# kamperh/segmentalist

Hardware: AMD Instinct MI355X
Metric: Gibbs sweeps/sec (10k utts, D=100, K=1000) at 1/2/4/8 MI355X (higher is better)
Workload: dtype fp16 one-product filter + fp16x2 second stage, float32 reference arithmetic for the results; 1 GPU; SegmentalKMeansWordseg batch-synchronous sweep (BASELINE.json configs[2]); utterances=10000, landmarks_per_utt=20, n_slices_max=6, embeddings=1050000, D=100, K=1000, parallelism=utterance shards x1, ONE all-gather of the packed block statistics per sweep, collective=none (single process), sweep_launch=plain launches, corpus=one device holds all rows, device_memory_allocated_bytes_rank0=1237140992, components_after=815

## Files before the change

### segmentalist_amd/csrc/segk_score_hint.hip

```cpp
#include "segk_kmeans_dev.h"

#define SEGK_K1_NW 4
#define SEGK_HINT_CHUNK 8

#ifndef SEGK_K1_ABL
#define SEGK_K1_ABL 0
#endif

struct K1Set {
    const float *tiles;
    int n_tiles;
    int tpr, n_ranges;
    float2 *part;
    int grid;
};

struct HintArgs {
    const unsigned char *ximg;
    const int32_t *ids;
    int64_t row0, n;
    K1Set full, delta;
    int K_max;
    int dbg;
    unsigned long long *stamp;
    float *fb_w;
    unsigned int *fb_t;
    int fb_cur;
    const int32_t *remap;
    int32_t *zero_cnt, *pre_hdr;
    int64_t k1_groups;
    const float *xrows32;
    int64_t ld32;
    const float *means32;
    const int32_t *cand_k;
    const float *nxx;
    float4 *hint_out;
    int32_t *ctl;
    const int32_t *meanchg;
    float *snap_img;
};

#define SEGK_MEANCHG_BIT 0x40000000

#define SEGK_RS_DRAIN_QUAD(O_, AO, q_, FIRST)                                                                               \
    do {                                                                                                                     \
        float x1_, u_;                                                                                                       \
        if (FIRST) {                                                                                                         \
            const float t1_ = __builtin_amdgcn_fmed3f(m1[O_], AO[4 * (q_)], AO[4 * (q_) + 1]);                              \
            asm volatile("v_max3_f32 %2, %0, %4, %5\n\t"                                                                     \
                         "v_med3_f32 %3, %2, %6, %7\n\t"                                                                     \
                         "v_max3_f32 %0, %2, %6, %7\n\t"                                                                     \
                         "v_max3_f32 %1, %1, %8, %3"                                                                          \
                         : "+v"(m1[O_]), "+v"(m2[O_]), "=&v"(x1_), "=&v"(u_)                                                 \
                         : "v"(AO[4 * (q_)]), "v"(AO[4 * (q_) + 1]), "v"(AO[4 * (q_) + 2]), "v"(AO[4 * (q_) + 3]), "v"(t1_)); \
        } else {                                                                                                             \
            float t1_;                                                                                                       \
            asm volatile("v_med3_f32 %4, %0, %5, %6\n\t"                                                                     \
                         "v_max3_f32 %2, %0, %5, %6\n\t"                                                                     \
                         "v_med3_f32 %3, %2, %7, %8\n\t"                                                                     \
                         "v_max3_f32 %0, %2, %7, %8\n\t"                                                                     \
                         "v_max3_f32 %1, %1, %4, %3"                                                                          \
                         : "+v"(m1[O_]), "+v"(m2[O_]), "=&v"(x1_), "=&v"(u_), "=&v"(t1_)                                     \
                         : "v"(AO[4 * (q_)]), "v"(AO[4 * (q_) + 1]), "v"(AO[4 * (q_) + 2]), "v"(AO[4 * (q_) + 3]));         \
        }                                                                                                                    \
    } while (0)

template <int KS, int V>
__device__ __forceinline__ void hint_wave_rows(const HintArgs &H, const int32_t *map , int64_t w, int64_t n_w, bool skip_ok)
{
    constexpr int D = 16 * KS - 4 * V;
    constexpr int nfull = D & ~7, nblk = nfull >> 3, rem = D & 7;
    constexpr int NX = nblk + (rem ? 1 : 0);
    typedef float f32x4_t __attribute__((ext_vector_type(4)));
    typedef float f32x2_t __attribute__((ext_vector_type(2)));
    typedef const __attribute__((address_space(1))) f32x4_t *gptr_t;
    const int lane = threadIdx.x & 63, row = lane >> 1, h = lane & 1;
    auto pk_sub = [](f32x2_t a, f32x2_t b2) -> f32x2_t {
        f32x2_t d;
        asm("v_pk_add_f32 %0, %1, %2 neg_lo:[0,1] neg_hi:[0,1]" : "=v"(d) : "v"(a), "v"(b2));
        return d;
    };
    const int64_t n_steps = (H.n + 31) >> 5;
    if (H.dbg & 8) return;
    auto rid_of = [&](int64_t s_) -> int32_t {
        const int64_t p_ = s_ * 32 + row;
        return p_ < H.n ? (H.ids ? H.ids[p_] : (int32_t)(H.row0 + p_)) : -1;
    };
    auto step_body = [&](int64_t s, int32_t rid_c, int32_t hint, bool skip, auto &&mid) {
        f32x4_t xv[NX], mv[NX];
#pragma unroll
        for (int b = 0; b < NX; b++) { xv[b] = f32x4_t{0.f, 0.f, 0.f, 0.f}; mv[b] = xv[b]; }
        if (!skip) {
            int64_t r_any = rid_c >= 0 ? (int64_t)rid_c : (H.ids ? 0 : H.row0);
            if (H.dbg & 16) r_any &= 1023;
            const uintptr_t xa = (uintptr_t)(H.xrows32 + r_any * H.ld32);
            const uintptr_t ma = (uintptr_t)(H.means32 + (int64_t)(hint >= 0 ? hint : 0) * D);
#pragma unroll
            for (int b = 0; b < nblk; b++) xv[b] = *reinterpret_cast<gptr_t>(xa + 16u * h + 32u * b);
            if constexpr (rem != 0) xv[nblk] = *reinterpret_cast<gptr_t>(xa + 4u * nfull);
#pragma unroll
            for (int b = 0; b < nblk; b++) mv[b] = *reinterpret_cast<gptr_t>(ma + 16u * h + 32u * b);
            if constexpr (rem != 0) mv[nblk] = *reinterpret_cast<gptr_t>(ma + 4u * nfull);
        }
        const float nx = rid_c >= 0 ? H.nxx[rid_c] : 0.f;
        if (H.dbg & 64) __builtin_amdgcn_s_sleep(64);
        mid();
        f32x2_t rl = {0.f, 0.f}, rh = {0.f, 0.f};
#pragma unroll
        for (int b = 0; b < ((H.dbg & 32) ? 1 : nblk); b++) {
            const f32x2_t dl = pk_sub(mv[b].xy, xv[b].xy), dh = pk_sub(mv[b].zw, xv[b].zw);
            const f32x2_t tl = dl * dl, th = dh * dh;
            rl = b == 0 ? tl : rl + tl;
            rh = b == 0 ? th : rh + th;
        }
        float res = (rl.x + rl.y) + (rh.x + rh.y);
        const float ro = __shfl_xor(res, 1);
        res = (h == 0) ? res + ro : ro + res;
        if constexpr (rem != 0) {
            const f32x2_t dl = pk_sub(mv[nblk].xy, xv[nblk].xy), dh = pk_sub(mv[nblk].zw, xv[nblk].zw);
            const f32x2_t tl = dl * dl, th = dh * dh;
            res += tl.x;
            if (rem > 1) res += tl.y;
            if (rem > 2) res += th.x;
            if (rem > 3) res += th.y;
        }
        const float sc = -res;
        const int64_t p = s * 32 + row;
        if (h == 0 && p < H.n && !skip) H.hint_out[p] = make_float4(sc, 0.5f * (sc - nx), __int_as_float(rid_c >= 0 ? hint : -1), 0.f);
    };
    int n_skipped = 0;
    if (skip_ok) {
        constexpr int CH = SEGK_HINT_CHUNK, PPL = CH / 2;
        const int crow = lane & 31, chalf = lane >> 5;
        auto chunk_load = [&](int64_t s0, int32_t (&rd)[PPL], int32_t (&kp)[PPL], int32_t (&pzv)[PPL]) {
#pragma unroll
            for (int u = 0; u < PPL; u++) {
                const int64_t s_ = s0 + (int64_t)(2 * u + chalf) * n_w, p_ = s_ * 32 + crow;
                const bool in = s_ < n_steps && p_ < H.n;
                rd[u] = in ? (H.ids ? H.ids[p_] : (int32_t)(H.row0 + p_)) : -1;
                pzv[u] = in ? __float_as_int(H.hint_out[p_].z) : -2;
            }
#pragma unroll
            for (int u = 0; u < PPL; u++) kp[u] = rd[u] >= 0 ? H.cand_k[rd[u]] : -1;
        };
        for (int64_t s0 = w; s0 < n_steps; s0 += (int64_t)CH * n_w) {
            int32_t rd[PPL], hv[PPL];
            unsigned long long live[PPL];
            {
                int32_t kp[PPL], pzv[PPL];
                chunk_load(s0, rd, kp, pzv);
#pragma unroll
                for (int u = 0; u < PPL; u++) {
                    const int64_t s_ = s0 + (int64_t)(2 * u + chalf) * n_w;
                    const bool in = s_ < n_steps && s_ * 32 + crow < H.n;
                    int32_t hint = (rd[u] >= 0 && kp[u] >= 0 && kp[u] < H.K_max) ? map[kp[u]] : -1;
                    const bool mchg = hint >= 0 && (hint & SEGK_MEANCHG_BIT) != 0;
                    if (hint >= 0) hint &= ~SEGK_MEANCHG_BIT;
                    const bool skip = rd[u] >= 0 && hint >= 0 && !mchg && pzv[u] == hint;
                    hv[u] = skip ? (hint | SEGK_MEANCHG_BIT) : hint;
                    live[u] = __ballot(in && !skip);
                    n_skipped += __popcll(__ballot(skip));
                }
            }
#pragma unroll 1
            for (int i = 0; i < CH; i++) {
                const int64_t s_ = s0 + (int64_t)i * n_w;
                if (s_ >= n_steps) break;
                int32_t rd_s = rd[0], hv_s = hv[0];
                unsigned long long lv = live[0];
#pragma unroll
                for (int u = 1; u < PPL; u++)
                    if ((i >> 1) == u) { rd_s = rd[u]; hv_s = hv[u]; lv = live[u]; }
                const int sh = 32 * (i & 1);
                if ((unsigned)(lv >> sh) == 0u) continue;
                const int src = sh + row;
                const int32_t rid_c = __shfl(rd_s, src);
                int32_t hint = __shfl(hv_s, src);
                const bool skip = hint >= 0 && (hint & SEGK_MEANCHG_BIT) != 0;
                if (hint >= 0) hint &= ~SEGK_MEANCHG_BIT;
                step_body(s_, rid_c, rid_c >= 0 ? hint : -1, skip, [] {});
            }
        }
        if (n_skipped > 0 && lane == 0) atomicAdd(H.ctl + 3, n_skipped);
        return;
    }
    int64_t s = w;
    int32_t rid = -1, rid_n = -1, kprev = -1;
    if (s < n_steps) {
        rid = rid_of(s);
        if (s + n_w < n_steps) rid_n = rid_of(s + n_w);
        kprev = rid >= 0 ? H.cand_k[rid] : -1;
    }
    for (; s < n_steps; s += n_w) {
        int32_t hint = (rid >= 0 && kprev >= 0 && kprev < H.K_max) ? map[kprev] : -1;
        if (hint >= 0) hint &= ~SEGK_MEANCHG_BIT;
        step_body(s, rid, hint, false, [&] {
            rid = rid_n;
            kprev = rid >= 0 ? H.cand_k[rid] : -1;
            const int64_t s2 = s + 2 * n_w;
            rid_n = s2 < n_steps ? rid_of(s2) : -1;
        });
    }
}

struct XcdShare { int64_t lo, hi; };
__device__ __forceinline__ XcdShare k1_xcd_share(const HintArgs &H, int64_t total_groups, bool delta, bool record)
{
    const int lane = threadIdx.x & 63, x = lane & 7;
    const int cur = H.fb_cur, prev = (cur + 2) % 3, next = (cur + 1) % 3;
    const float wp = H.fb_w[prev * 8 + x];
    const unsigned int tp = H.fb_t ? H.fb_t[prev * 8 + x] : 0u;
    const bool ok = __all(tp > 0u && wp > 0.f);
    const float rate = ok ? wp / (float)tp : 0.f;
    float rsum = rate;
    rsum += __shfl_xor(rsum, 1);
    rsum += __shfl_xor(rsum, 2);
    rsum += __shfl_xor(rsum, 4);
    float w = !(wp > 0.f) ? 0.125f : ok ? 0.5f * wp + 0.5f * (rate / rsum) : wp;
    w = fminf(fmaxf(w, 0.0625f), 0.25f);
    float wsum = w;
    wsum += __shfl_xor(wsum, 1);
    wsum += __shfl_xor(wsum, 2);
    wsum += __shfl_xor(wsum, 4);
    double cum = 0.0;
    for (int y = 0; y < 8; y++) {
        const float wy = __shfl(w, y);
        if (y < x) cum += (double)wy;
    }
    const int64_t split = (int64_t)(cum * ((double)total_groups / (double)wsum));
    const int xcd = blockIdx.x & 7;
    XcdShare s;
    s.lo = __shfl(split, xcd);
    s.hi = xcd == 7 ? total_groups : __shfl(split, (xcd + 1) & 7);
    if (record && lane < 8) {
        H.fb_w[cur * 8 + x] = delta ? (wp > 0.f ? wp : 0.125f) : w / wsum;
        if (H.fb_t) {
            H.fb_t[next * 8 + x] = 0u;
            if (delta) H.fb_t[cur * 8 + x] = tp;
        }
    }
    return s;
}

template <int KS, int V>
__global__ __launch_bounds__(128 * SEGK_K1_NW, 1) void k_kmeans_top2_rs(HintArgs H)
{
    typedef _Float16 T;
    typedef SegkPiece::V8 V8;
    constexpr int P = 2, KP = KS * 16, NBLK = 2;
    constexpr int STRIDE = (KS * P * 256 + 32 + 1023) / 1024 * 1024;
    constexpr int TL = KS * 256 + 32;
    extern __shared__ __attribute__((aligned(16))) float lds[];
    const int tid = threadIdx.x, lane = tid & 63, wave = tid >> 6;
    const int j = lane & 31, h = lane >> 5;
    const int mw = H.ctl ? __builtin_amdgcn_readfirstlane(H.ctl[0]) : 0;
    const bool delta = (mw & SEGK_DELTA_MODE) != 0, skip_ok = (mw & SEGK_DELTA_SKIP) != 0;
    const K1Set S = delta ? H.delta : H.full;
    const int n_tiles = delta ? __builtin_amdgcn_readfirstlane(H.ctl[2]) : S.n_tiles;
    const int tpr = S.tpr, R = S.n_ranges, grid = S.grid;
    const float *tiles = S.tiles;
    float2 *part = S.part;
    if ((int)blockIdx.x >= grid) return;
    const int map_off = tpr * TL;
    const bool is_hint = wave >= SEGK_K1_NW;
    if (!is_hint) __builtin_amdgcn_s_setprio(2);
#ifdef SEGK_STAMP
    const unsigned long long st_k0 = __builtin_amdgcn_s_memtime(), st_r0 = __builtin_amdgcn_s_memrealtime();
#endif
    int range, wgr, n_wgr;
    const bool xcd_aware = (grid & 7) == 0 && ((grid >> 3) % R) == 0;
    if (xcd_aware) {
        const int xcd = blockIdx.x & 7, idx = blockIdx.x >> 3;
        range = idx % R;
        wgr = (idx / R) * 8 + xcd;
        n_wgr = grid / R;
    } else {
        n_wgr = grid / R;
        range = blockIdx.x % R;
        wgr = blockIdx.x / R;
    }
    const int t_lo = range * tpr;
    int nt = n_tiles - t_lo;
    if (nt > tpr) nt = tpr;
    const bool mm_on = wgr < n_wgr && nt > 0;
    if (nt < 1) nt = 1;
    const T *plane0 = (const T *)(H.ximg + SEGK_SP_HEADER);
    const int64_t total_groups = (H.n + 32 * NBLK - 1) / (32 * NBLK);
    int64_t n_groups = H.k1_groups < total_groups ? H.k1_groups : total_groups, n_slots = (int64_t)n_wgr * SEGK_K1_NW, g_first = (int64_t)wgr * SEGK_K1_NW + wave;
    const unsigned long long fb_t0 = __builtin_amdgcn_s_memrealtime();
    if (blockIdx.x == 0 && tid == 0) {
        if (H.zero_cnt) *H.zero_cnt = 0;
#pragma unroll
        for (int i = 0; i < 16; i++) H.pre_hdr[i] = 0;
    }
    const XcdShare share = k1_xcd_share(H, total_groups, delta, blockIdx.x == 0 && wave == 0);
    const bool fb = xcd_aware && H.fb_t != nullptr && !delta;
    if (fb) {
        n_slots = (int64_t)(n_wgr >> 3) * SEGK_K1_NW;
        g_first = share.lo + (int64_t)(wgr >> 3) * SEGK_K1_NW + wave;
        n_groups = share.hi;
    }

#define SEGK_RS_LOAD(g_, XB)                                                                                    \
    do {                                                                                                         \
        _Pragma("unroll") for (int b = 0; b < NBLK; b++) {                                                       \
            const int64_t r = (g_) * (32 * NBLK) + 32 * b + j;                                                   \
            int64_t rowid = -1;                                                                                  \
            if (r < H.n) rowid = H.ids ? (int64_t)H.ids[r] : H.row0 + r;                                         \
            if (rowid < 0) rowid = 0;           \
            const T *xp = plane0 + rowid * KP + 8 * h;                                                           \
            _Pragma("unroll") for (int s = 0; s < KS; s++) XB[b][s] = *reinterpret_cast<const V8 *>(xp + 16 * s); \
        }                                                                                                        \
    } while (0)

#define SEGK_RS_UNIT(XB, N_, AN, O_, AO, REFILL)                                                                     \
    do {                                                                                                              \
        _Pragma("unroll") for (int s = 0; s < KS; s++) {                                                              \
            asm volatile("" : "+v"(a[s]));                                                                            \
            AN = __builtin_amdgcn_mfma_f32_32x32x16_f16(a[s], XB[N_][s], s == 0 ? cs : AN, 0, 0, 0);                  \
            asm volatile("" : "+v"(AN));                                                                              \
            if (REFILL && !(SEGK_K1_ABL & 2)) {    \
                load_a(tn, s);                                                                                        \
                if (s == 0) load_cs(tn);                                                                              \
            }                                                                                                         \
            __builtin_amdgcn_sched_barrier(0);                                                                        \
                      \
            constexpr int SL = KS > 1 ? KS - 1 : 1;                                                                   \
            const int q_lo = KS > 1 ? ((s - 1) * 4 + SL - 1) / SL : 0, q_hi = KS > 1 ? (s * 4 + SL - 1) / SL : 4;     \
            if ((KS == 1 || s >= 1) && !(SEGK_K1_ABL & 1)) {                                                          \
                if (0 >= q_lo && 0 < q_hi) SEGK_RS_DRAIN_QUAD(O_, AO, 0, true);                                       \
                if (1 >= q_lo && 1 < q_hi) SEGK_RS_DRAIN_QUAD(O_, AO, 1, false);                                      \
                if (2 >= q_lo && 2 < q_hi) SEGK_RS_DRAIN_QUAD(O_, AO, 2, false);                                      \
                if (3 >= q_lo && 3 < q_hi) SEGK_RS_DRAIN_QUAD(O_, AO, 3, false);                                      \
            }                                                                                                         \
            __builtin_amdgcn_sched_barrier(0);                                                                        \
        }                                                                                                             \
    } while (0)

#define SEGK_RS_TILE(XB, t_)                                        \
    do {                                                            \
        const int tn = (t_) + 1 < nt ? (t_) + 1 : 0;      \
        SEGK_RS_UNIT(XB, 0, acc0, 1, acc1, false);                  \
        SEGK_RS_UNIT(XB, 1, acc1, 0, acc0, true);                   \
    } while (0)

#define SEGK_RS_GROUP(g_, XB)                                                                                             \
    do {                                                                                                                   \
        float m1[NBLK], m2[NBLK];                                                                                          \
        _Pragma("unroll") for (int b = 0; b < NBLK; b++) { m1[b] = NEG_INF_F; m2[b] = NEG_INF_F; }                         \
        f32x16 acc0, acc1;                                                                                                 \
        _Pragma("unroll") for (int q = 0; q < 16; q++) acc1[q] = NEG_INF_F;         \
        int t = 0;                                                                                                         \
        for (; t + 1 < nt; t += 2) {                                                                                       \
            SEGK_RS_TILE(XB, t);                                                                                           \
            SEGK_RS_TILE(XB, t + 1);                                                                                       \
        }                                                                                                                  \
        if (t < nt) SEGK_RS_TILE(XB, t);                                                                                   \
        SEGK_RS_DRAIN_QUAD(NBLK - 1, acc1, 0, true);                                                                       \
        SEGK_RS_DRAIN_QUAD(NBLK - 1, acc1, 1, false);                                                                      \
        SEGK_RS_DRAIN_QUAD(NBLK - 1, acc1, 2, false);                                                                      \
        SEGK_RS_DRAIN_QUAD(NBLK - 1, acc1, 3, false);                                                                      \
           \
          \
          \
        _Pragma("unroll") for (int b = 0; b < NBLK; b++) {                                                                 \
            const float o1 = __shfl_xor(m1[b], 32), o2 = __shfl_xor(m2[b], 32);                                            \
            pend1[b] = fmaxf(m1[b], o1);                                                                                   \
            pend2[b] = fmaxf(fminf(m1[b], o1), fmaxf(m2[b], o2));                                                          \
        }                                                                                                                  \
        pend_g = (g_);                                                                                                     \
    } while (0)

#define SEGK_RS_STORE()                                                                                                    \
    do {                                                                                                                   \
        if (pend_g >= 0) {                                                                                                 \
            _Pragma("unroll") for (int b = 0; b < NBLK; b++) {                                                             \
                const int64_t r = pend_g * (32 * NBLK) + 32 * b + j;                                                       \
                if (h == 0 && r < H.n && !(H.dbg & 1)) part[(int64_t)range * H.n + r] = make_float2(pend1[b], pend2[b]); \
            }                                                                                                              \
        }                                                                                                                  \
    } while (0)

    V8 a[KS];
    f32x16 cs;
    auto load_a = [&](int t, int s) { a[s] = *reinterpret_cast<const V8 *>((const T *)(lds + t * TL) + (s * 64 + lane) * 8); };
    auto load_cs = [&](int t) {
        const float *cv = lds + t * TL + KS * 256 + 4 * h;
#pragma unroll
        for (int q = 0; q < 4; q++) {
            const float4 c4 = *reinterpret_cast<const float4 *>(cv + 8 * q);
            cs[4 * q + 0] = c4.x; cs[4 * q + 1] = c4.y; cs[4 * q + 2] = c4.z; cs[4 * q + 3] = c4.w;
        }
    };
    int64_t g = g_first;
    float pend1[NBLK], pend2[NBLK];
    int64_t pend_g = -1;
    V8 xa[NBLK][KS];
    typedef __attribute__((address_space(3))) void *lptr_t;
    if (!is_hint && mm_on && g < n_groups && !(H.dbg & 4)) SEGK_RS_LOAD(g, xa);
#ifdef SEGK_STAMP
    const unsigned long long st_k1 = __builtin_amdgcn_s_memtime();
#endif
    {
        constexpr int MAXT = (160 * 1024 / (TL * 4)) < SEGK_HINT_MAX_TPR ? (160 * 1024 / (TL * 4)) : SEGK_HINT_MAX_TPR;
        constexpr int MAXB = MAXT * KS;
        constexpr int NWF = 2 * SEGK_K1_NW;
        constexpr int PER_W = (MAXB + NWF - 1) / NWF;
        const int n_blk = nt * KS;
        const int rot = (int)(((unsigned)wgr * 2654435761u) >> 8) % n_blk;
        const unsigned lds0 = __builtin_amdgcn_readfirstlane((unsigned)(uintptr_t)(lptr_t)lds);
#pragma unroll
        for (int u = 0; u < PER_W; u++) {
            int c = wave + u * NWF;
            if (mm_on && c < n_blk) {
                c += rot;
                if (c >= n_blk) c -= n_blk;
                const int t = __builtin_amdgcn_readfirstlane(c / KS), ks = __builtin_amdgcn_readfirstlane(c) - t * KS;
                const float *src = tiles + (int64_t)(t_lo + t) * STRIDE + ks * (P * 256) + lane * 4;
                const unsigned dst = lds0 + (unsigned)(t * TL + ks * 256) * 4u;
                unsigned keep_;
                asm volatile("s_mov_b32 %0, m0\n\ts_mov_b32 m0, %2\n\ts_nop 0\n\t"
                             "global_load_lds_dwordx4 %1, off\n\ts_mov_b32 m0, %0"
                             : "=&s"(keep_)
                             : "v"(src), "s"(dst)
                             : "memory");
            }
        }
        float4 cv4 = make_float4(0.f, 0.f, 0.f, 0.f);
        const bool has_c = mm_on && tid < nt * 8;
        if (has_c) cv4 = *reinterpret_cast<const float4 *>(tiles + (int64_t)(t_lo + (tid >> 3)) * STRIDE + KS * P * 256 + (tid & 7) * 4);
        int32_t *map_l = reinterpret_cast<int32_t *>(lds + map_off);
        for (int k = tid; k < H.K_max; k += 128 * SEGK_K1_NW) {
            int v = H.remap ? H.remap[k] : k;
            if (v < 0 || v >= H.K_max) v = -1;
            else if (H.full.tiles[(int64_t)(v >> 5) * STRIDE + KS * P * 256 + (v & 31)] < -1.0e37f) v = -1;
            if (skip_ok && v >= 0 && H.meanchg[v]) v |= SEGK_MEANCHG_BIT;
            map_l[k] = v;
        }
        if (has_c) *reinterpret_cast<float4 *>(lds + (tid >> 3) * TL + KS * 256 + (tid & 7) * 4) = cv4;
        static_assert(128 * SEGK_K1_NW >= MAXT * 8, "one thread per float4 of the constants");
    }
    asm volatile("s_waitcnt vmcnt(0)" ::: "memory");
    __syncthreads();
    if (is_hint) {
        if (H.ctl && !delta && mm_on && wgr == 0) {
            float4 *dst = reinterpret_cast<float4 *>(H.snap_img + 4 + (int64_t)t_lo * TL);
            const float4 *src = reinterpret_cast<const float4 *>(lds);
            for (int i = tid - 64 * SEGK_K1_NW; i < nt * (TL / 4); i += 64 * SEGK_K1_NW) dst[i] = src[i];
        }
        hint_wave_rows<KS, V>(H, reinterpret_cast<const int32_t *>(lds + map_off), (int64_t)blockIdx.x * SEGK_K1_NW + (wave - SEGK_K1_NW),
                              (int64_t)grid * SEGK_K1_NW, skip_ok);
        return;
    }
#ifdef SEGK_STAMP
    const unsigned long long st_k2 = __builtin_amdgcn_s_memtime();
#endif
    if (!mm_on || g >= n_groups || (H.dbg & 128)) return;
    if (H.dbg & 4) SEGK_RS_LOAD(g, xa);
#pragma unroll
    for (int s = 0; s < KS; s++) load_a(0, s);
    load_cs(0);
    V8 xb[NBLK][KS];
#ifdef SEGK_STAMP
    unsigned long long st_wait = 0, st_loop = 0, st_groups = 0;
    const unsigned long long st_begin = __builtin_amdgcn_s_memtime();
#define SEGK_ST(var) const unsigned long long var = __builtin_amdgcn_s_memtime()
#else
#define SEGK_ST(var) do { } while (0)
#endif
    for (;;) {
        SEGK_ST(s0);
        __builtin_amdgcn_s_waitcnt(0x0F70);
        SEGK_ST(s1);
        const int64_t g1 = g + n_slots;
        if (g1 < n_groups) SEGK_RS_LOAD(g1, xb);
        SEGK_RS_STORE();
        SEGK_ST(s2);
        SEGK_RS_GROUP(g, xa);
        SEGK_ST(s3);
#ifdef SEGK_STAMP
        st_wait += s1 - s0; st_loop += s3 - s2; st_groups++;
#endif
        if (g1 >= n_groups) break;
        SEGK_ST(s4);
        __builtin_amdgcn_s_waitcnt(0x0F70);
        SEGK_ST(s5);
        g = g1 + n_slots;
        if (g < n_groups) SEGK_RS_LOAD(g, xa);
        SEGK_RS_STORE();
        SEGK_ST(s6);
        SEGK_RS_GROUP(g1, xb);
        SEGK_ST(s7);
#ifdef SEGK_STAMP
        st_wait += s5 - s4; st_loop += s7 - s6; st_groups++;
#endif
        if (g >= n_groups) break;
    }
#ifdef SEGK_STAMP
    if (H.stamp && lane == 0) {
        unsigned long long *o = H.stamp + ((int64_t)blockIdx.x * SEGK_K1_NW + wave) * 8;
        o[0] = st_wait; o[1] = st_loop; o[2] = __builtin_amdgcn_s_memtime() - st_begin; o[3] = st_groups;
        o[4] = st_begin - st_k0; o[5] = st_r0; o[6] = __builtin_amdgcn_s_memrealtime(); o[7] = ((st_k1 - st_k0) << 32) | (st_k2 - st_k1);
    }
#endif
#undef SEGK_ST
    SEGK_RS_STORE();
    if (fb && lane == 0) atomicMax(&H.fb_t[H.fb_cur * 8 + (blockIdx.x & 7)], (unsigned int)(__builtin_amdgcn_s_memrealtime() - fb_t0));
#undef SEGK_RS_STORE
#undef SEGK_RS_GROUP
#undef SEGK_RS_TILE
#undef SEGK_RS_UNIT
#undef SEGK_RS_LOAD
}
#undef SEGK_RS_DRAIN_QUAD

template <int KS>
__global__ __launch_bounds__(SEGK_PREP_THREADS) void k_delta_prep(DeltaPrepArgs P)
{
    if ((int)blockIdx.x >= P.n_tiles) {
        delta_prep_means_rows(P, (int)blockIdx.x - P.n_tiles, (int)gridDim.x - P.n_tiles);
        return;
    }
    __shared__ DeltaPrepLds S;
    const int e_cur = ((const int *)P.tiles_hdr)[0];
    if (delta_prep_tile(P, KS, (int)blockIdx.x, e_cur, S)) delta_prep_mode(P, KS, e_cur, S);
}

struct HintMergeArgs {
    const float2 *part;
    const float4 *hint_out;
    int n_ranges;
    const float *tiles_hdr;
    const unsigned char *ximg;
    const int32_t *ctl;
    const float2 *part_delta;
    int32_t *lab_base;
    const int32_t *colchg;
    const int32_t *meanchg;
    int32_t *lab_last;
    int32_t *stats_host;
};

#define SEGK_MERGE_ROWS 6144
#define SEGK_MERGE_THREADS 1024
__global__ __launch_bounds__(SEGK_MERGE_THREADS) void k_hint_merge(ScoreArgs A, HintMergeArgs H, int KP, int64_t per, float *pre_thr, int64_t first_skipped)
{
    __shared__ int32_t ulist[SEGK_MERGE_ROWS];
    __shared__ float uthr[SEGK_MERGE_ROWS];
    __shared__ int32_t ucnt, ubase;
    const int tid = threadIdx.x, lane = tid & 63;
    if (tid == 0) ucnt = 0;
    const int mw = H.ctl ? H.ctl[0] : 0;
    const bool delta = (mw & SEGK_DELTA_MODE) != 0;
    const int n_chg = H.ctl ? H.ctl[1] : 0, n_packed = H.ctl ? H.ctl[2] : 0;
    if (H.stats_host && blockIdx.x == 0 && tid == 0) {
        H.stats_host[1] = n_chg;
        H.stats_host[2] = n_packed;
        H.stats_host[3] = H.ctl ? H.ctl[3] : 0;
        __hip_atomic_store(H.stats_host, H.ctl ? 1 + (delta ? 1 : 0) : 0, __ATOMIC_RELEASE, __HIP_MEMORY_SCOPE_SYSTEM);
    }
    __syncthreads();
    bool carry = false;
    if (delta && (mw & SEGK_DELTA_SKIP) != 0 && H.lab_last) {
        const int c_off = (KP / 16) * 512;
        bool bad = false;
        for (int k = tid; k < A.K_max; k += SEGK_MERGE_THREADS)
            if (H.meanchg[k] && !H.colchg[k])
                bad |= !(H.tiles_hdr[1024 + (int64_t)(k >> 5) * A.tile_stride + c_off + (k & 31)] < -1.0e37f);
        carry = __syncthreads_or(bad ? 1 : 0) == 0;
    }
    const int64_t p_lo = (int64_t)blockIdx.x * per, p_hi = p_lo + per < A.n ? p_lo + per : A.n;
    const int e_ab = ((const int *)H.ximg)[1] + ((const int *)H.tiles_hdr)[0];
    const float unscale = ldexpf(1.f, -e_ab), scale = ldexpf(1.f, e_ab);
    const float M = (float)(sqrt(*A.mnorm2) * (1.0 + 1e-6)) + 1e-30f;
    const float Em = H.tiles_hdr[1];
    constexpr int U = 5;
    for (int64_t p0 = p_lo; p0 < p_hi; p0 += SEGK_MERGE_THREADS * U) {
        int32_t rid[U];
        float4 ho[U];
        float t1[U], t2[U], xnb[U], xer[U], d1[U];
        int32_t last[U];
        bool cw[U];
#pragma unroll
        for (int j = 0; j < U; j++) {
            const int64_t p = p0 + j * SEGK_MERGE_THREADS + tid;
            rid[j] = -1;
            if (p < p_hi) rid[j] = A.ids ? A.ids[p] : (int32_t)(A.row0 + p);
        }
#pragma unroll
        for (int j = 0; j < U; j++) {
            const int64_t p = p0 + j * SEGK_MERGE_THREADS + tid;
            ho[j] = make_float4(0.f, 0.f, __int_as_float(-1), 0.f);
            t1[j] = NEG_INF_F; t2[j] = NEG_INF_F; xnb[j] = 0.f; xer[j] = 0.f;
            if (rid[j] >= 0) {
                ho[j] = H.hint_out[p];
                for (int r = 0; r < H.n_ranges; r++) {
                    const float2 pv = H.part[(int64_t)r * A.n + p];
                    const float n1 = fmaxf(t1[j], pv.x);
                    t2[j] = fmaxf(fminf(t1[j], pv.x), fmaxf(t2[j], pv.y));
                    t1[j] = n1;
                }
                xnb[j] = A.xnorm[rid[j]];
                xer[j] = A.xerr[rid[j]];
            }
            d1[j] = NEG_INF_F;
            last[j] = -2;
            cw[j] = false;
            if (rid[j] >= 0 && carry) {
                const int32_t hint = __float_as_int(ho[j].z);
                last[j] = H.lab_last[p];
                cw[j] = hint >= 0 && last[j] == hint && H.meanchg[hint] == 0;
            }
            if (rid[j] >= 0 && delta) {
                const int32_t hint = __float_as_int(ho[j].z);
                if (hint >= 0 && H.colchg[hint] && H.lab_base[p] == hint) {
                    t1[j] = t2[j];
                }
                if (n_packed > 0) {
                    const float2 pv = H.part_delta[p];
                    d1[j] = pv.x;
                    const float n1 = fmaxf(t1[j], pv.x);
                    t2[j] = fmaxf(fminf(t1[j], pv.x), fmaxf(t2[j], pv.y));
                    t1[j] = n1;
                }
            }
        }
#pragma unroll
        for (int j = 0; j < U; j++) {
            bool und = false;
            float thr = 0.f;
            int32_t keep = -1;
            if (rid[j] >= 0 && p0 + j * SEGK_MERGE_THREADS + tid >= first_skipped) {
                const int q2 = atomicAdd(A.cand.count, 1);
                if (q2 < A.amb_cap) A.cand.queue[q2] = rid[j];
            } else if (rid[j] >= 0) {
                const int32_t hint = __float_as_int(ho[j].z);
                und = true;
                const float tau = filter_tau_h1(xnb[j], M, A.D, xer[j], Em);
                float lower = t1[j];
                thr = t1[j] - tau * scale * 1.000001f;
                thr -= 4e-7f * fabsf(t1[j]);
                bool ok = false;
                if (hint >= 0) {
                    const float top1 = t1[j] * unscale, top2 = t2[j] * unscale;
                    const float u = 5.9604645e-8f;
                    const float e1 = (1.02f * (float)(KP + 16) + 16.f) * u * (xnb[j] * M + 0.5f * M * M);
                    const float rnd = 1.00001f * fminf((xnb[j] + xer[j]) * Em + xer[j] * M, 1.01f * 9.765625e-4f * xnb[j] * M);
                    const float s2 = xnb[j] + M;
                    const float dl = ((float)(A.D / 8 + 13) + 4.f) * u * s2 * s2;
                    ok = (top1 - top2 > tau) && (ho[j].y >= top1 - tau + (e1 + rnd + dl) * 1.0001f);
                    const bool carried = !ok && cw[j] && ho[j].y > d1[j] * unscale + (e1 + rnd + dl) * 1.0001f;
                    if (ok || carried) {
                        A.cand.k[rid[j]] = hint;
                        A.cand.s[rid[j]] = (double)ho[j].x;
                        und = false;
                        keep = hint;
                    }
                    lower = (ho[j].y - (e1 + rnd + dl) * 1.0001f) * scale;
                    lower -= 4e-7f * fabsf(lower);
                }
                if (H.lab_base && !delta) H.lab_base[p0 + j * SEGK_MERGE_THREADS + tid] = ok ? hint : -1;
                if (und && delta && n_chg > 0) {
                    if (hint < 0) {
                        und = false;
                        const int q2 = atomicAdd(A.cand.count, 1);
                        if (q2 < A.amb_cap) A.cand.queue[q2] = rid[j];
                    } else {
                        lower = fmaxf(lower, d1[j]);
                        thr = lower - tau * scale * 1.000001f;
                        thr -= 4e-7f * fabsf(lower);
                    }
                }
            }
            if (H.lab_last && rid[j] >= 0 && last[j] != keep) H.lab_last[p0 + j * SEGK_MERGE_THREADS + tid] = keep;
            const unsigned long long mask = __ballot(und);
            if (mask != 0ull) {
                const int before = __builtin_amdgcn_mbcnt_hi((unsigned)(mask >> 32), __builtin_amdgcn_mbcnt_lo((unsigned)mask, 0));
                int base = 0;
                if (lane == 0) base = atomicAdd(&ucnt, __popcll(mask));
                base = __shfl(base, 0);
                if (und) {
                    ulist[base + before] = rid[j];
                    uthr[base + before] = thr;
                }
            }
        }
    }
    __syncthreads();
    const int cnt = ucnt;
    if (cnt == 0) return;
    if (tid == 0) ubase = atomicAdd(A.pre_count, cnt);
    __syncthreads();
    const int base = ubase;
    for (int i = tid; i < cnt; i += SEGK_MERGE_THREADS) {
        const int q = base + i;
        const int32_t rid = ulist[i];
        if (q < A.pre_cap) {
            A.pre_queue[q] = rid;
            if (pre_thr) pre_thr[q] = uthr[i];
        } else {
            const int q2 = atomicAdd(A.cand.count, 1);
            if (q2 < A.amb_cap) A.cand.queue[q2] = rid;
        }
    }
}

struct HintLaunch {
    HintPlan lds;
    bool band;
    int grid;
    int64_t k1_groups;
    float *fb_w;
    unsigned int *fb_t;
    int fb_cur;
    float4 *hint_out;
    bool part_fresh;
};

static int hint_workspaces(segk_ctx *ctx, ScoreArgs &A, HintLaunch &L, hipStream_t st)
{
    if (int rc = segk_ws_grow(ctx, &ctx->pre_queue, &ctx->pre_cap, A.n, sizeof(int32_t) * (size_t)(A.n + 16), st)) return rc;
    A.pre_queue = ctx->pre_queue + 16;
    A.pre_count = ctx->pre_queue;
    A.pre_cap = (int)A.n;
    if (L.band)
        if (int rc = segk_ws_grow(ctx, &ctx->pre_thr, &ctx->pre_thr_cap, A.n, sizeof(float) * (size_t)A.n, st)) return rc;
    const size_t part_bytes = ((size_t)L.lds.n_ranges * (size_t)A.n * sizeof(float2) + 255) & ~(size_t)255;
    const size_t need_part = part_bytes + (size_t)A.n * sizeof(float4);
    L.part_fresh = ctx->hint_part_bytes < need_part;
    if (int rc = segk_ws_grow(ctx, &ctx->hint_part, &ctx->hint_part_bytes, need_part, need_part, st)) return rc;
    L.hint_out = (float4 *)((unsigned char *)ctx->hint_part + part_bytes);
    if (!ctx->hint_fb) {
        float init[3 * 8 + 3 * 8];
        SEGK_CHECK_HIP(hipMalloc(&ctx->hint_fb, sizeof(init)));
        for (int i = 0; i < 24; i++) init[i] = 0.125f;
        memset(init + 24, 0, 24 * sizeof(unsigned int));
        SEGK_CHECK_HIP(hipMemcpyAsync(ctx->hint_fb, init, sizeof(init), hipMemcpyHostToDevice, st));
        SEGK_CHECK_HIP(hipStreamSynchronize(st));
        ctx->hint_fb_launch = 0;
    }
    return SEGK_OK;
}

static void hint_plan_rows(segk_ctx *ctx, const ScoreArgs &A, HintLaunch &L)
{
    const int n_ranges = L.lds.n_ranges;
    const int64_t total_groups = (A.n + 63) / 64;
    L.fb_w = (float *)ctx->hint_fb;
    const bool fb_big = total_groups >= 192 * 64;
    L.fb_t = (segk_env_int("SEGK_HINT_BALANCE", 1) == 0 || !fb_big) ? nullptr : (unsigned int *)(L.fb_w + 24);
    L.fb_cur = (int)(ctx->hint_fb_launch++ % 3u);
    L.grid = (ctx->n_cu / n_ranges) * n_ranges;
    const int64_t steps = (A.n + 64 * SEGK_K1_NW - 1) / (64 * SEGK_K1_NW);
    if ((int64_t)L.grid / n_ranges > steps) L.grid = (int)steps * n_ranges;
    L.k1_groups = total_groups;
    if (!L.fb_t && !L.band) {
        const int64_t slots = (int64_t)(L.grid / n_ranges) * SEGK_K1_NW;
        const int64_t whole = slots > 0 ? (total_groups / slots) * slots : 0;
        if (whole > 0 && total_groups - whole <= 32) L.k1_groups = whole;
    }
}

struct DeltaBuf {
    int32_t *ctl;
    int32_t *colchg, *meanchg;
    float *snap_img;
    float *packed;
    float *snap_means;
    float2 *part;
    int32_t *lab_base;
    int32_t *lab_last;
    size_t zero_bytes;
};
static size_t delta_layout(unsigned char *b, int n_tiles, int K_max, int D, int64_t n, int stride, DeltaBuf *B)
{
    const size_t TL = (size_t)(segk_b3_kp(D) / 16) * 256 + 32;
    size_t off = 0;
    auto take = [&](size_t bytes) {
        unsigned char *p = b ? b + off : nullptr;
        off += (bytes + 255) & ~(size_t)255;
        return p;
    };
    B->ctl = (int32_t *)take(256);
    B->colchg = (int32_t *)take((size_t)n_tiles * 32 * 4);
    B->meanchg = (int32_t *)take((size_t)K_max * 4);
    B->snap_img = (float *)take(((size_t)n_tiles * TL + 4) * 4);
    B->packed = (float *)take((size_t)n_tiles * stride * 4);
    B->zero_bytes = off;
    B->snap_means = (float *)take((size_t)K_max * D * 4);
    B->part = (float2 *)take((size_t)n * 8);
    B->lab_base = (int32_t *)take((size_t)n * 4);
    B->lab_last = (int32_t *)take((size_t)n * 4);
    return off;
}

static int delta_cap(const HintPlan &lds)
{
    int cap = segk_env_int("SEGK_DELTA_CAP", lds.tpr);
    if (cap > lds.max_tiles) cap = lds.max_tiles;
    return cap < 1 ? 1 : cap;
}
static int delta_budget(int n_tiles) { return segk_env_int("SEGK_DELTA_BUDGET", n_tiles); }

static DeltaPrepArgs delta_prep_args(segk_ctx *ctx, const DeltaBuf &B, const float *tiles, int n_tiles, int stride, int K_max, int D,
                                     const float *means32, const int32_t *remap, const int32_t *K_dev, bool valid, int cap, int budget,
                                     int redo_seq = -1)
{
    DeltaPrepArgs P{};
    P.tiles_hdr = tiles; P.n_tiles = n_tiles; P.stride = stride;
    P.K_max = K_max; P.D = D; P.means32 = means32; P.remap = remap; P.K_dev = K_dev;
    P.valid = valid ? 1 : 0; P.hint_valid = valid ? 1 : 0; P.cap = cap;
    P.budget = budget;
    P.redo = redo_seq >= 0 ? 1 : 0;
    P.seq = redo_seq >= 0 ? redo_seq : (int)(ctx->delta_seq++ & 1u);
    P.ctl = B.ctl; P.colchg = B.colchg; P.meanchg = B.meanchg;
    P.snap_img = B.snap_img; P.packed = B.packed; P.snap_means = B.snap_means;
    return P;
}

bool segk_delta_prep_fold(segk_ctx *ctx, const segk_corpus *c, const segk_kmeans *m, const int32_t *remap, hipStream_t st, DeltaPrepArgs *P)
{
    *P = DeltaPrepArgs{};
    if (!ctx || ctx->delta_pending != 0 || !ctx->delta_valid || ctx->capturing || !ctx->delta_buf) return false;
    if (segk_env_int("SEGK_DELTA_PREP_FOLD", 1) == 0 || segk_env_int("SEGK_SCORE_DELTA", 1) == 0) return false;
    const void *key[4] = {c->Xb3, c->X32, m->tiles_b3, m->means};
    const int64_t key_n[5] = {0, c->n_emb, c->n_emb, m->K_max, c->D};
    if (memcmp(key, ctx->delta_key, sizeof(key)) != 0 || memcmp(key_n, ctx->delta_key_n, sizeof(key_n)) != 0) return false;
    const int n_tiles = segk_n_tiles(m->K_max), stride_sp = segk_sp_tile_stride(c->D, 2);
    HintPlan lds;
    if (n_tiles > 32 * SEGK_PREP_COLS || !segk_hint_plan(m->K_max, segk_b3_kp(c->D) / 16, n_tiles, &lds)) return false;
    DeltaBuf B{};
    if (ctx->delta_bytes != delta_layout(nullptr, n_tiles, m->K_max, c->D, c->n_emb, stride_sp, &B)) return false;
    delta_layout((unsigned char *)ctx->delta_buf, n_tiles, m->K_max, c->D, c->n_emb, stride_sp, &B);
    const int cap = delta_cap(lds), budget = delta_budget(n_tiles);
    *P = delta_prep_args(ctx, B, m->tiles_b3, n_tiles, stride_sp, m->K_max, c->D, (const float *)m->means, remap, m->K, true, cap, budget);
    ctx->delta_pending = 1;
    ctx->delta_pending_remap = remap; ctx->delta_pending_K = m->K; ctx->delta_pending_stream = (const void *)st;
    ctx->delta_pending_cap = cap; ctx->delta_pending_budget = budget; ctx->delta_pending_seq = P->seq;
    return true;
}

template <int KS>
static int launch_delta_prep(segk_ctx *ctx, const ScoreArgs &A, const int32_t *remap, const int32_t *K_dev, int64_t n_emb,
                             const HintLaunch &L, hipStream_t st, DeltaBuf *B, int *cap)
{
    *B = DeltaBuf{};
    *cap = 0;
    const int pending = ctx->delta_pending;
    ctx->delta_pending = 0;
    const bool delta_on = segk_env_int("SEGK_SCORE_DELTA", 1) != 0 && L.band && A.ids == nullptr && A.n_tiles <= 32 * SEGK_PREP_COLS;
    const void *key[6] = {A.X32, A.xrows32, A.tiles, A.means32, A.cand.k, A.cand.s};
    const int64_t key_n[5] = {A.row0, A.n, n_emb, A.K_max, A.D};
    bool state_valid = delta_on && !L.part_fresh && ctx->delta_valid && memcmp(key, ctx->delta_key, sizeof(key)) == 0 &&
                       memcmp(key_n, ctx->delta_key_n, sizeof(key_n)) == 0;
    ctx->delta_valid = 0;
    if (!delta_on) return SEGK_OK;
    const int stride_sp = segk_sp_tile_stride(A.D, 2);
    const size_t need = delta_layout(nullptr, A.n_tiles, A.K_max, A.D, A.n, stride_sp, B);
    if (ctx->delta_bytes != need) {
        ctx->delta_bytes = 0;
        if (int rc = segk_ws_realloc(ctx, &ctx->delta_buf, need, st)) return rc;
        ctx->delta_bytes = need;
        state_valid = false;
        SEGK_CHECK_HIP(hipMemsetAsync(ctx->delta_buf, 0, B->zero_bytes, st));
    }
    delta_layout((unsigned char *)ctx->delta_buf, A.n_tiles, A.K_max, A.D, A.n, stride_sp, B);
    *cap = delta_cap(L.lds);
    const int budget = delta_budget(A.n_tiles);
    const bool folded = pending == 1 && state_valid && remap == ctx->delta_pending_remap && K_dev == ctx->delta_pending_K &&
                        (const void *)st == ctx->delta_pending_stream && *cap == ctx->delta_pending_cap &&
                        budget == ctx->delta_pending_budget;
    if (!folded) {
        const DeltaPrepArgs P = delta_prep_args(ctx, *B, A.tiles, A.n_tiles, stride_sp, A.K_max, A.D, A.means32, remap, K_dev, state_valid,
                                                *cap, budget, pending != 0 && state_valid ? ctx->delta_pending_seq : -1);
        hipLaunchKernelGGL(k_delta_prep<KS>, dim3(A.n_tiles + segk_delta_prep_row_blocks(A.K_max)), dim3(SEGK_PREP_THREADS), 0, st, P);
    }
    memcpy(ctx->delta_key, key, sizeof(key));
    memcpy(ctx->delta_key_n, key_n, sizeof(key_n));
    ctx->delta_valid = 1;
    return SEGK_OK;
}

template <int KS>
static int launch_k1(segk_ctx *ctx, const ScoreArgs &A, const int32_t *remap, int64_t n_emb, const HintLaunch &L, const DeltaBuf &B,
                     int delta_cap, hipStream_t st)
{
    constexpr int TL = KS * 256 + 32;
    HintArgs H{};
    H.ximg = (const unsigned char *)A.X32;
    H.ids = A.ids; H.row0 = A.row0; H.n = A.n;
    H.K_max = A.K_max;
    H.dbg = segk_dev_env("SEGK_HINT_DBG");
#ifdef SEGK_STAMP
    H.stamp = getenv("SEGK_STAMP_PTR") ? (unsigned long long *)strtoull(getenv("SEGK_STAMP_PTR"), nullptr, 0) : nullptr;
#endif
    H.fb_w = L.fb_w; H.fb_t = L.fb_t; H.fb_cur = L.fb_cur;
    H.remap = remap;
    H.zero_cnt = ctx->defer_zero;
    ctx->defer_zero = nullptr;
    H.pre_hdr = ctx->pre_queue;
    H.k1_groups = L.k1_groups;
    H.xrows32 = A.xrows32; H.ld32 = A.ld32; H.means32 = A.means32;
    H.cand_k = A.cand.k;
    H.nxx = A.xerr + n_emb;
    H.hint_out = L.hint_out;
    H.ctl = B.ctl; H.meanchg = B.meanchg; H.snap_img = B.snap_img;
    H.full = K1Set{A.tiles + 1024, A.n_tiles, L.lds.tpr, L.lds.n_ranges, (float2 *)ctx->hint_part, L.grid};
    size_t lds = (size_t)L.lds.tpr * TL * sizeof(float) + L.lds.map_bytes;
    int grid = L.grid;
    if (B.ctl) {
        const int64_t steps = (A.n + 64 * SEGK_K1_NW - 1) / (64 * SEGK_K1_NW);
        H.delta = K1Set{B.packed, 0, delta_cap, 1, B.part, (int64_t)ctx->n_cu > steps ? (int)steps : ctx->n_cu};
        const size_t lds_d = (size_t)delta_cap * TL * sizeof(float) + L.lds.map_bytes;
        if (H.delta.grid > grid) grid = H.delta.grid;
        if (lds_d > lds) lds = lds_d;
    }
    const bool prof = segk_prof_now(ctx);
    const int slot = ctx->prof_n % SEGK_PROF_SLOTS;
#define SEGK_K1_LAUNCH(VV)                                                                                                  \
    do {                                                                                                                     \
        SEGK_CHECK_HIP(segk_dyn_lds((const void *)k_kmeans_top2_rs<KS, VV>, lds));                                           \
        if (prof) SEGK_CHECK_HIP(hipEventRecord(ctx->prof_ev[slot][0], st));                                                 \
        hipLaunchKernelGGL((k_kmeans_top2_rs<KS, VV>), dim3((unsigned)grid), dim3(128 * SEGK_K1_NW), lds, st, H);            \
    } while (0)
    switch ((16 * KS - A.D) / 4) {
        case 0: SEGK_K1_LAUNCH(0); break;
        case 1: SEGK_K1_LAUNCH(1); break;
        case 2: SEGK_K1_LAUNCH(2); break;
        default: SEGK_K1_LAUNCH(3); break;
    }
#undef SEGK_K1_LAUNCH
    if (prof) {
        SEGK_CHECK_HIP(hipEventRecord(ctx->prof_ev[slot][1], st));
        ctx->prof_rows[slot] = A.n;
        ctx->prof_kind = 5;
        ctx->prof_launches = 1;
        ctx->prof_n++;
    }
    return SEGK_OK;
}

static void launch_merge(segk_ctx *ctx, const ScoreArgs &A, const HintLaunch &L, const DeltaBuf &B, int ks, hipStream_t st)
{
    HintMergeArgs E{};
    E.part = (const float2 *)ctx->hint_part;
    E.hint_out = L.hint_out;
    E.n_ranges = L.lds.n_ranges;
    E.tiles_hdr = A.tiles;
    E.ximg = (const unsigned char *)A.X32;
    E.ctl = B.ctl;
    E.part_delta = B.part;
    E.lab_base = B.lab_base;
    E.colchg = B.colchg;
    E.meanchg = B.meanchg;
    E.lab_last = B.lab_last;
    E.stats_host = ctx->delta_host_dev;
    int64_t grid = (int64_t)ctx->n_cu;
    if (grid * SEGK_MERGE_THREADS > A.n) grid = (A.n + SEGK_MERGE_THREADS - 1) / SEGK_MERGE_THREADS;
    if (grid * SEGK_MERGE_ROWS < A.n) grid = (A.n + SEGK_MERGE_ROWS - 1) / SEGK_MERGE_ROWS;
    const int64_t per = (A.n + grid - 1) / grid;
    hipLaunchKernelGGL(k_hint_merge, dim3((unsigned)grid), dim3(SEGK_MERGE_THREADS), 0, st, A, E, ks * 16, per,
                       L.band ? ctx->pre_thr : nullptr, L.k1_groups * 64);
}

template <int KS>
static int launch_score_hint(segk_ctx *ctx, ScoreArgs A, const int32_t *remap, const int32_t *K_dev, int64_t n_emb, hipStream_t st)
{
    HintLaunch L{};
    L.band = segk_band_applies(A);
    SEGK_REQUIRE(segk_hint_plan(A.K_max, KS, A.n_tiles, &L.lds),
                 "hinted score path: K_max too large for K1's LDS (the label map beside four ranges of tile images at most)");
    if (int rc = hint_workspaces(ctx, A, L, st)) return rc;
    hint_plan_rows(ctx, A, L);
    DeltaBuf B;
    int delta_cap;
    if (int rc = launch_delta_prep<KS>(ctx, A, remap, K_dev, n_emb, L, st, &B, &delta_cap)) return rc;
    if (int rc = launch_k1<KS>(ctx, A, remap, n_emb, L, B, delta_cap, st)) return rc;
    launch_merge(ctx, A, L, B, KS, st);
    if (L.band) return segk_launch_band(ctx, A, ctx->pre_thr, A.n, B.lab_last, KS, st);
    ScoreArgs B2 = A;
    B2.ids = A.pre_queue;
    B2.row0 = 0;
    B2.n = A.n;
    B2.n_dev = ctx->pre_queue;
    if (int rc = segk_launch_sp_second(ctx, B2, KS, st)) return rc;
    SEGK_LAUNCH_CHECK();
    return SEGK_OK;
}

int segk_dispatch_score_hint(segk_ctx *ctx, const ScoreArgs &A, const int32_t *remap, const int32_t *K_dev, int64_t n_emb, int ks, hipStream_t st)
{
    switch (ks) {
        case 1: return launch_score_hint<1>(ctx, A, remap, K_dev, n_emb, st);
        case 2: return launch_score_hint<2>(ctx, A, remap, K_dev, n_emb, st);
        case 3: return launch_score_hint<3>(ctx, A, remap, K_dev, n_emb, st);
        case 4: return launch_score_hint<4>(ctx, A, remap, K_dev, n_emb, st);
        case 5: return launch_score_hint<5>(ctx, A, remap, K_dev, n_emb, st);
        case 6: return launch_score_hint<6>(ctx, A, remap, K_dev, n_emb, st);
        case 7: return launch_score_hint<7>(ctx, A, remap, K_dev, n_emb, st);
        case 8: return launch_score_hint<8>(ctx, A, remap, K_dev, n_emb, st);
        default: break;
    }
    segk_set_error("hinted score path: D out of range");
    return SEGK_ERR_UNSUPPORTED;
}
```

Baseline: 7216 sweeps/s.

## Compact live hint rows across chunks and prefetch next chunk metadata

Result: faster. 7396 sweeps/s, median of 6 (+2.5%).

```diff
diff --git a/segmentalist_amd/csrc/segk_score_hint.hip b/segmentalist_amd/csrc/segk_score_hint.hip
--- a/segmentalist_amd/csrc/segk_score_hint.hip
+++ b/segmentalist_amd/csrc/segk_score_hint.hip
@@ -86,7 +86,7 @@
         const int64_t p_ = s_ * 32 + row;
         return p_ < H.n ? (H.ids ? H.ids[p_] : (int32_t)(H.row0 + p_)) : -1;
     };
-    auto step_body = [&](int64_t s, int32_t rid_c, int32_t hint, bool skip, auto &&mid) {
+    auto step_body = [&](int64_t p, int32_t rid_c, int32_t hint, bool skip, auto &&mid) {
         f32x4_t xv[NX], mv[NX];
 #pragma unroll
         for (int b = 0; b < NX; b++) { xv[b] = f32x4_t{0.f, 0.f, 0.f, 0.f}; mv[b] = xv[b]; }
@@ -125,14 +125,13 @@
             if (rem > 3) res += th.y;
         }
         const float sc = -res;
-        const int64_t p = s * 32 + row;
         if (h == 0 && p < H.n && !skip) H.hint_out[p] = make_float4(sc, 0.5f * (sc - nx), __int_as_float(rid_c >= 0 ? hint : -1), 0.f);
     };
     int n_skipped = 0;
     if (skip_ok) {
         constexpr int CH = SEGK_HINT_CHUNK, PPL = CH / 2;
         const int crow = lane & 31, chalf = lane >> 5;
-        auto chunk_load = [&](int64_t s0, int32_t (&rd)[PPL], int32_t (&kp)[PPL], int32_t (&pzv)[PPL]) {
+        auto chunk_load = [&](int64_t s0, int32_t (&rd)[PPL], int32_t (&kp)[PPL], int32_t (&pzv)[PPL]) __attribute__((always_inline)) {
 #pragma unroll
             for (int u = 0; u < PPL; u++) {
                 const int64_t s_ = s0 + (int64_t)(2 * u + chalf) * n_w, p_ = s_ * 32 + crow;
@@ -143,44 +142,92 @@
 #pragma unroll
             for (int u = 0; u < PPL; u++) kp[u] = rd[u] >= 0 ? H.cand_k[rd[u]] : -1;
         };
+        auto sel_bit = [](unsigned w_, int n_) __attribute__((always_inline)) -> int {
+            int base = 0;
+#pragma unroll
+            for (int sh = 16; sh >= 1; sh >>= 1) {
+                const int t = __popc(w_ & ((1u << sh) - 1u));
+                const bool up = n_ >= t;
+                w_ = up ? w_ >> sh : w_;
+                base += up ? sh : 0;
+                n_ -= up ? t : 0;
+            }
+            return base & 31;
+        };
+        int c_n = 0;
+        int64_t c_p = 0;
+        int32_t c_rid = -1, c_hint = -1;
+        int32_t rd_n[PPL], kp_n[PPL], pz_n[PPL];
+        chunk_load(w, rd_n, kp_n, pz_n);
         for (int64_t s0 = w; s0 < n_steps; s0 += (int64_t)CH * n_w) {
             int32_t rd[PPL], hv[PPL];
             unsigned long long live[PPL];
+            int pre[PPL + 1];
+            pre[0] = 0;
+#pragma unroll
+            for (int u = 0; u < PPL; u++) {
+                const int64_t s_ = s0 + (int64_t)(2 * u + chalf) * n_w;
+                const bool in = s_ < n_steps && s_ * 32 + crow < H.n;
+                rd[u] = rd_n[u];
+                int32_t hint = (rd[u] >= 0 && kp_n[u] >= 0 && kp_n[u] < H.K_max) ? map[kp_n[u]] : -1;
+                const bool mchg = hint >= 0 && (hint & SEGK_MEANCHG_BIT) != 0;
+                if (hint >= 0) hint &= ~SEGK_MEANCHG_BIT;
+                const bool skip = rd[u] >= 0 && hint >= 0 && !mchg && pz_n[u] == hint;
+                hv[u] = hint;
+                live[u] = __ballot(in && !skip);
+                pre[u + 1] = pre[u] + __popcll(live[u]);
+                n_skipped += __popcll(__ballot(skip));
+            }
+            const int64_t s1 = s0 + (int64_t)CH * n_w;
+            chunk_load(s1, rd_n, kp_n, pz_n);
+            if (pre[PPL] == 0) continue;
+            const int total = c_n + pre[PPL];
+            auto fetch = [&](int g0, int64_t &p_e, int32_t &rid_e, int32_t &hint_e) __attribute__((always_inline)) -> bool {
+                const int g_ = g0 + row, j_ = g_ - c_n;
+                unsigned w_ = (unsigned)live[0];
+                int i_ = 0, jj = j_;
+#pragma unroll
+                for (int i = 1; i < CH; i++) {
+                    const int at = (i & 1) ? pre[i >> 1] + __popc((unsigned)live[i >> 1]) : pre[i >> 1];
+                    const unsigned wi = (i & 1) ? (unsigned)(live[i >> 1] >> 32) : (unsigned)live[i >> 1];
+                    const bool up = j_ >= at;
+                    w_ = up ? wi : w_;
+                    i_ = up ? i : i_;
+                    jj = up ? j_ - at : jj;
+                }
+                const int src = 32 * (i_ & 1) + sel_bit(w_, jj);
+                int32_t r_ = __shfl(rd[0], src), h_ = __shfl(hv[0], src);
+#pragma unroll
+                for (int u = 1; u < PPL; u++) {
+                    const int32_t ru = __shfl(rd[u], src), hu = __shfl(hv[u], src);
+                    const bool up = j_ >= pre[u];
+                    r_ = up ? ru : r_;
+                    h_ = up ? hu : h_;
+                }
+                const int64_t s_ = s0 + (int64_t)i_ * n_w;
+                const bool carried = j_ < 0;
+                p_e = carried ? c_p : s_ * 32 + (src & 31);
+                rid_e = carried ? c_rid : r_;
+                hint_e = carried ? c_hint : (r_ >= 0 ? h_ : -1);
+                return g_ < total;
+            };
+            int done = 0;
+#pragma unroll 1
+            for (; total - done >= 32; done += 32) {
+                int64_t p_e;
+                int32_t rid_e, hint_e;
+                fetch(done, p_e, rid_e, hint_e);
+                step_body(p_e, rid_e, hint_e, false, [] {});
+            }
             {
-                int32_t kp[PPL], pzv[PPL];
-                chunk_load(s0, rd, kp, pzv);
-#pragma unroll
-                for (int u = 0; u < PPL; u++) {
-                    const int64_t s_ = s0 + (int64_t)(2 * u + chalf) * n_w;
-                    const bool in = s_ < n_steps && s_ * 32 + crow < H.n;
-                    int32_t hint = (rd[u] >= 0 && kp[u] >= 0 && kp[u] < H.K_max) ? map[kp[u]] : -1;
-                    const bool mchg = hint >= 0 && (hint & SEGK_MEANCHG_BIT) != 0;
-                    if (hint >= 0) hint &= ~SEGK_MEANCHG_BIT;
-                    const bool skip = rd[u] >= 0 && hint >= 0 && !mchg && pzv[u] == hint;
-                    hv[u] = skip ? (hint | SEGK_MEANCHG_BIT) : hint;
-                    live[u] = __ballot(in && !skip);
-                    n_skipped += __popcll(__ballot(skip));
-                }
+                int64_t p_e;
+                int32_t rid_e, hint_e;
+                const bool on = fetch(done, p_e, rid_e, hint_e);
+                c_p = p_e; c_rid = on ? rid_e : -1; c_hint = on ? hint_e : -1;
+                c_n = total - done;
             }
-#pragma unroll 1
-            for (int i = 0; i < CH; i++) {
-                const int64_t s_ = s0 + (int64_t)i * n_w;
-                if (s_ >= n_steps) break;
-                int32_t rd_s = rd[0], hv_s = hv[0];
-                unsigned long long lv = live[0];
-#pragma unroll
-                for (int u = 1; u < PPL; u++)
-                    if ((i >> 1) == u) { rd_s = rd[u]; hv_s = hv[u]; lv = live[u]; }
-                const int sh = 32 * (i & 1);
-                if ((unsigned)(lv >> sh) == 0u) continue;
-                const int src = sh + row;
-                const int32_t rid_c = __shfl(rd_s, src);
-                int32_t hint = __shfl(hv_s, src);
-                const bool skip = hint >= 0 && (hint & SEGK_MEANCHG_BIT) != 0;
-                if (hint >= 0) hint &= ~SEGK_MEANCHG_BIT;
-                step_body(s_, rid_c, rid_c >= 0 ? hint : -1, skip, [] {});
-            }
-        }
+        }
+        if (c_n > 0) step_body(c_p, c_rid, c_hint, row >= c_n, [] {});
         if (n_skipped > 0 && lane == 0) atomicAdd(H.ctl + 3, n_skipped);
         return;
     }
@@ -194,7 +241,7 @@
     for (; s < n_steps; s += n_w) {
         int32_t hint = (rid >= 0 && kprev >= 0 && kprev < H.K_max) ? map[kprev] : -1;
         if (hint >= 0) hint &= ~SEGK_MEANCHG_BIT;
-        step_body(s, rid, hint, false, [&] {
+        step_body(s * 32 + row, rid, hint, false, [&] {
             rid = rid_n;
             kprev = rid >= 0 ? H.cand_k[rid] : -1;
             const int64_t s2 = s + 2 * n_w;
```
